# showlab/VideoSwap

Measured on NVIDIA H100. Metric: denoise-steps/sec, 16f 512^2 SD1.5 UNet3D (CFG UNet fwd + CFG combine + DDIM step), higher is better.
Workload: dtype f16

## Files before the change

videoswap_b200/csrc/common.cuh:

```cuda
#pragma once
#include <cuda.h>
#include <cuda_fp16.h>
#include <cuda_runtime.h>
#include <stdint.h>
#include <stdio.h>

namespace vs {

void set_error(const char* fmt, ...);
const char* last_error();

#define VS_CHECK_CUDA(expr)                                                                         \
  do {                                                                                              \
    cudaError_t _e = (expr);                                                                        \
    if (_e != cudaSuccess) {                                                                        \
      vs::set_error("%s:%d CUDA error %s: %s", __FILE__, __LINE__, #expr, cudaGetErrorString(_e)); \
      return 1;                                                                                     \
    }                                                                                               \
  } while (0)

#define VS_REQUIRE(cond, ...)                \
  do {                                       \
    if (!(cond)) {                           \
      vs::set_error(__VA_ARGS__);            \
// ... 41 lines not shown
  ProfScope(cudaStream_t st, int cat, double work, int nlaunch = 1, long long m = 0, int n = 0, int k = 0);
  ~ProfScope();
  cudaStream_t st_; int idx_;
};
void prof_enable(bool on);
void prof_reset();
int prof_collect(int cat, double* ms, double* work, long long* count);
int prof_dump(const char* path);
long long launch_count();
void count_launch(int n);

#ifdef __CUDACC__
__device__ __forceinline__ uint32_t smem_u32(const void* p) { return (uint32_t)__cvta_generic_to_shared(p); }

__device__ __forceinline__ void mbar_init(uint32_t bar, uint32_t count) {
  asm volatile("mbarrier.init.shared::cta.b64 [%0], %1;" ::"r"(bar), "r"(count) : "memory");
}
__device__ __forceinline__ void fence_barrier_init() {
  asm volatile("fence.mbarrier_init.release.cluster;" ::: "memory");
}
__device__ __forceinline__ void fence_proxy_async() { asm volatile("fence.proxy.async.shared::cta;" ::: "memory"); }
__device__ __forceinline__ void mbar_expect_tx(uint32_t bar, uint32_t bytes) {
  asm volatile("mbarrier.arrive.expect_tx.shared::cta.b64 _, [%0], %1;" ::"r"(bar), "r"(bytes) : "memory");
}
__device__ __forceinline__ void mbar_arrive(uint32_t bar) {
  asm volatile("mbarrier.arrive.shared::cta.b64 _, [%0];" ::"r"(bar) : "memory");
}
__device__ __forceinline__ bool mbar_try_wait(uint32_t bar, uint32_t parity) {
  uint32_t ok;
  asm volatile(
      "{\n\t.reg .pred p;\n\t"
      "mbarrier.try_wait.parity.shared::cta.b64 p, [%1], %2;\n\t"
      "selp.u32 %0, 1, 0, p;\n\t}"
      : "=r"(ok)
      : "r"(bar), "r"(parity)
      : "memory");
  return ok != 0;
}
__device__ __forceinline__ void mbar_wait(uint32_t bar, uint32_t parity) {
  if (mbar_try_wait(bar, parity)) return;
  uint32_t spins = 0;
  while (!mbar_try_wait(bar, parity)) {
    if (++spins > (1u << 25)) __trap();
  }
}

__device__ __forceinline__ void prefetch_tmap(const CUtensorMap* m) {
  asm volatile("prefetch.tensormap [%0];" ::"l"(reinterpret_cast<uint64_t>(m)) : "memory");
}
__device__ __forceinline__ void tma_load_2d(uint32_t dst, const CUtensorMap* m, uint32_t bar, int c0, int c1) {
  asm volatile(
      "cp.async.bulk.tensor.2d.shared::cluster.global.mbarrier::complete_tx::bytes [%0], [%1, {%3, %4}], [%2];"
      ::"r"(dst), "l"(reinterpret_cast<uint64_t>(m)), "r"(bar), "r"(c0), "r"(c1)
      : "memory");
}
__device__ __forceinline__ void tma_load_4d(uint32_t dst, const CUtensorMap* m, uint32_t bar, int c0, int c1, int c2,
                                            int c3) {
  asm volatile(
      "cp.async.bulk.tensor.4d.shared::cluster.global.mbarrier::complete_tx::bytes [%0], [%1, {%3, %4, %5, %6}], [%2];"
      ::"r"(dst), "l"(reinterpret_cast<uint64_t>(m)), "r"(bar), "r"(c0), "r"(c1), "r"(c2), "r"(c3)
      : "memory");
}

__device__ __forceinline__ bool elect_one() {
  uint32_t pred;
  asm volatile(
      "{\n\t.reg .pred P;\n\t"
      "elect.sync _|P, 0xffffffff;\n\t"
      "selp.u32 %0, 1, 0, P;\n\t}"
      : "=r"(pred));
  return pred != 0;
}

__device__ __forceinline__ uint32_t cluster_ctarank() {
  uint32_t r;
  asm volatile("mov.u32 %0, %%cluster_ctarank;" : "=r"(r));
  return r;
}
__device__ __forceinline__ void cluster_sync_all() {
  asm volatile("barrier.cluster.arrive.release.aligned;" ::: "memory");
  asm volatile("barrier.cluster.wait.acquire.aligned;" ::: "memory");
}
__device__ __forceinline__ uint32_t mapa_shared(uint32_t addr, uint32_t rank) {
  uint32_t r;
  asm volatile("mapa.shared::cluster.u32 %0, %1, %2;" : "=r"(r) : "r"(addr), "r"(rank));
  return r;
}
__device__ __forceinline__ void named_bar_sync(int id, int nthreads) {
  asm volatile("bar.sync %0, %1;" ::"r"(id), "r"(nthreads) : "memory");
}
__device__ __forceinline__ void named_bar_arrive(int id, int nthreads) {
  asm volatile("bar.arrive %0, %1;" ::"r"(id), "r"(nthreads) : "memory");
}

__device__ __forceinline__ void pdl_trigger() { asm volatile("griddepcontrol.launch_dependents;" ::: "memory"); }
__device__ __forceinline__ void pdl_wait() { asm volatile("griddepcontrol.wait;" ::: "memory"); }

template <int N>
__device__ __forceinline__ void setmaxnreg_dec() { asm volatile("setmaxnreg.dec.sync.aligned.u32 %0;" ::"n"(N)); }
template <int N>
__device__ __forceinline__ void setmaxnreg_inc() { asm volatile("setmaxnreg.inc.sync.aligned.u32 %0;" ::"n"(N)); }

__device__ __forceinline__ void wgmma_fence() { asm volatile("wgmma.fence.sync.aligned;" ::: "memory"); }
__device__ __forceinline__ void wgmma_commit() { asm volatile("wgmma.commit_group.sync.aligned;" ::: "memory"); }
template <int N>
__device__ __forceinline__ void wgmma_wait() { asm volatile("wgmma.wait_group.sync.aligned %0;" ::"n"(N) : "memory"); }
// ... 112 lines not shown
```

videoswap_b200/csrc/gemm.cu:

```cuda
#include <type_traits>

#include "common.cuh"
#include "kernels.h"

namespace vs {

namespace {

constexpr int BM = 128;
constexpr int WG_M = 64;
constexpr int BK = 64;
constexpr int A_STAGE_BYTES = BM * BK * 2;
constexpr uint64_t A_HALF_DESC = (WG_M * BK * 2) >> 4;
constexpr int GEMM_THREADS = 384;
constexpr int SMEM_LIMIT = 227 * 1024;
constexpr int EPI_COLS = 32;
constexpr int EPI_WARP_BYTES = 16 * 64;
constexpr int EPI_BYTES = 8 * EPI_WARP_BYTES;
constexpr int PRODUCER_REGS = 40, CONSUMER_REGS = 232;
enum { EPI_F_GEGLU = 1, EPI_F_RES = 2, EPI_F_RV = 4, EPI_F_LN = 8, EPI_F_LNOUT = 16, EPI_F_QGELU = 32 };

struct GemmParams {
  CUtensorMap tmA, tmA2, tmB;
  int M, N;
  int num_kb;
  int kb_per_tap;
  int kb_src1;
  int taps;
  int a_rank;
  int nimg, H, W, TH, TW, TN, tiles_x, tiles_y;
  int tap_x0, tap_y0, tap_w;
  int osy, osx, ooy, oox, OH, OW;
  int tw_log, thw_log;
  int m_tiles, n_tiles;
  const float* bias;
  const float* rowvec;
  int ldrv;
  int pix_per_batch;
  int rv_mod;
  const float2* ln_stats;
  const float* ln_u;
  const float2* ln_parts;
  int ln_nparts;
  float ln_inv_c;
  float2* ln_sums_out;
  const __half* residual;
  int ldr;
  __half* out;
  int ldc;
  int staged;
  int stages;
};

struct GemmParamsSub : GemmParams {
  CUtensorMap tmS[3];
  int sub_short;
};

struct GemmParamsS2 : GemmParams {
  CUtensorMap tmP[3];
};

template <int BN>
struct Cfg {
  static constexpr bool COOP = BN > 160;
  static constexpr int HALVES = COOP ? 1 : 2;
  static constexpr int B_STAGE_BYTES = BN * BK * 2;
  static constexpr int STAGE_BYTES = A_STAGE_BYTES + B_STAGE_BYTES;
  static constexpr int STAGES_RAW = (SMEM_LIMIT - 2048 - EPI_BYTES) / STAGE_BYTES;
  static constexpr int STAGES = STAGES_RAW > 12 ? 12 : STAGES_RAW;
  static constexpr int SMEM_BYTES = STAGES * STAGE_BYTES + EPI_BYTES + 1024  + 256 ;
  static_assert(B_STAGE_BYTES % 1024 == 0, "B stage must keep 1024-byte alignment for SWIZZLE_128B");
  static_assert(STAGES >= 3, "pipeline too shallow");
  static_assert(BN % 32 == 0 && BN <= 256, "wgmma N");
};

__device__ __forceinline__ uint32_t sw64_off(int row, int chunk) {
  return (uint32_t)(row * 64 + ((chunk ^ ((row >> 1) & 3)) << 4));
}

template <int BN, int EPI, typename Params>
__global__ void __launch_bounds__(GEMM_THREADS, 1) gemm_tc_kernel(const __grid_constant__ Params p) {
  using C = Cfg<BN>;
  constexpr bool SUB = std::is_same<Params, GemmParamsSub>::value;
  constexpr bool S2 = std::is_same<Params, GemmParamsS2>::value;
  constexpr bool GEGLU = (EPI & EPI_F_GEGLU) != 0, HAS_RES = (EPI & EPI_F_RES) != 0, HAS_RV = (EPI & EPI_F_RV) != 0;
  constexpr bool LN = (EPI & EPI_F_LN) != 0;
  constexpr bool LNOUT = (EPI & EPI_F_LNOUT) != 0;
  constexpr bool QGELU = (EPI & EPI_F_QGELU) != 0;
  extern __shared__ uint8_t smem_raw[];
  const uint32_t smem_base = (smem_u32(smem_raw) + 1023u) & ~1023u;
  const uint32_t epi_base = smem_base + C::STAGES * C::STAGE_BYTES;
  const uint32_t bar_base = epi_base + EPI_BYTES;
  auto full_bar = [&](int s) { return bar_base + 8u * s; };
  auto empty_bar = [&](int s) { return bar_base + 8u * (C::STAGES + s); };

  const int warp = threadIdx.x >> 5;
  const int lane = threadIdx.x & 31;
  const int wg = threadIdx.x >> 7;
  const int nst = (p.stages > 0 && p.stages < C::STAGES) ? p.stages : C::STAGES;
  const int total_tiles = p.m_tiles * p.n_tiles;

  if (threadIdx.x == 0) {
    prefetch_tmap(&p.tmA);
    prefetch_tmap(&p.tmB);
    if (p.kb_src1 < p.kb_per_tap) prefetch_tmap(&p.tmA2);
    if constexpr (SUB) {
      if (p.sub_short & 1) prefetch_tmap(&p.tmS[0]);
      if (p.sub_short & 2) prefetch_tmap(&p.tmS[1]);
      if (p.sub_short == 3) prefetch_tmap(&p.tmS[2]);
    }
    if constexpr (S2) {
      for (int k = 0; k < 3; ++k) prefetch_tmap(&p.tmP[k]);
    }
    for (int s = 0; s < C::STAGES; ++s) {
      mbar_init(full_bar(s), 1);
      mbar_init(empty_bar(s), C::COOP ? 8 : 4);
    }
    fence_barrier_init();
  }
  __syncthreads();
  pdl_trigger();
  pdl_wait();

  if (wg == 0) {
    setmaxnreg_dec<PRODUCER_REGS>();
    if (warp != 0) return;
    const int num_kb = p.num_kb, kb_per_tap = p.kb_per_tap, kb_src1 = p.kb_src1;
    const bool conv = p.a_rank == 4;
    const int tap_x0 = p.tap_x0, tap_x1 = p.tap_x0 + p.tap_w;
    bool short_y = false, short_x = false;
    if constexpr (SUB) { short_y = (p.sub_short & 1) != 0; short_x = (p.sub_short & 2) != 0; }
    uint32_t pr_s = 0, pr_ph = 0;
    for (int t = blockIdx.x; t < total_tiles; t += gridDim.x) {
      const int m_tile = t / p.n_tiles, n_tile = t % p.n_tiles;
      int x0 = 0, y0 = 0, i0 = 0;
      if (conv) {
        x0 = (m_tile % p.tiles_x) * p.TW;
        y0 = ((m_tile / p.tiles_x) % p.tiles_y) * p.TH;
        i0 = (m_tile / (p.tiles_x * p.tiles_y)) * p.TN;
      }
      const int n0 = n_tile * BN;
      const int m0 = m_tile * BM;
      int kcoord = 0;
      int dy = p.tap_y0, dx = tap_x0;
      int r = 0;
      for (int kb = 0; kb < num_kb; ++kb) {
        mbar_wait(empty_bar(pr_s), pr_ph ^ 1);
        if (elect_one()) {
          const uint32_t fb = full_bar(pr_s);
          const uint32_t a_dst = smem_base + pr_s * C::STAGE_BYTES;
          const bool first = r < kb_src1;
          const CUtensorMap* tm = first ? &p.tmA : &p.tmA2;
          if constexpr (SUB) {
            const bool sy = short_y && dy == p.tap_y0 + 2, sx = short_x && dx == tap_x0 + 2;
            if (sy || sx) tm = sy ? (sx ? &p.tmS[2] : &p.tmS[0]) : &p.tmS[1];
          }
          int ox = dx, oy = dy;
          if constexpr (S2) {
            const int par = ((dy & 1) << 1) | (dx & 1);
            if (par) tm = &p.tmP[par - 1];
            ox = dx >> 1; oy = dy >> 1;
          }
          const int c = (first ? r : r - kb_src1) * BK;
          mbar_expect_tx(fb, C::STAGE_BYTES);
          if (conv) tma_load_4d(a_dst, tm, fb, c, x0 + ox, y0 + oy, i0);
          else tma_load_2d(a_dst, tm, fb, c, m0);
          tma_load_2d(a_dst + A_STAGE_BYTES, &p.tmB, fb, kcoord, n0);
        }
        __syncwarp();
        kcoord += BK;
        if (++r == kb_per_tap) {
          r = 0;
          if (++dx == tap_x1) { dx = tap_x0; ++dy; }
        }
        if (++pr_s == (uint32_t)nst) { pr_s = 0; pr_ph ^= 1; }
      }
    }
    return;
  }

  setmaxnreg_inc<CONSUMER_REGS>();
  const int g = wg - 1;
  const int wq = warp & 3;
  const int q = lane & 3;
  const int rbase = 16 * wq + (lane >> 2);
  const uint32_t stage_buf = epi_base + (uint32_t)(warp - 4) * EPI_WARP_BYTES;
  const bool has_bias = p.bias != nullptr;
  const bool staged = p.staged != 0;
  const int num_kb = p.num_kb;
  auto tile_pixel = [&](int m_tile, int row) -> int {
    if (p.a_rank == 4) {
      const int x0 = (m_tile % p.tiles_x) * p.TW;
      const int y0 = ((m_tile / p.tiles_x) % p.tiles_y) * p.TH;
      const int i0 = (m_tile / (p.tiles_x * p.tiles_y)) * p.TN;
      const int ti = row >> p.thw_log, rem = row & ((1 << p.thw_log) - 1);
      const int y = y0 + (rem >> p.tw_log), x = x0 + (rem & (p.TW - 1)), img = i0 + ti;
      if constexpr (SUB) {
        const int oy = y * p.osy + p.ooy, ox = x * p.osx + p.oox;
        return ((img < p.nimg) && (y < p.H) && (x < p.W) && (oy < p.OH) && (ox < p.OW)) ? (img * p.OH + oy) * p.OW + ox : -1;
      }
      return ((img < p.nimg) && (y < p.H) && (x < p.W)) ? (img * p.OH + y * p.osy + p.ooy) * p.OW + x * p.osx + p.oox : -1;
    }
    const int px = m_tile * BM + row;
    return px < p.M ? px : -1;
  };

  const int bar_mine = 1 + g, bar_other = 2 - g;
  float acc[C::HALVES][BN / 2];
  uint32_t s = 0, ph = 0;
  for (int t = blockIdx.x, j = 0; t < total_tiles; t += gridDim.x, ++j) {
    const int m_tile = t / p.n_tiles, n_tile = t % p.n_tiles;
    if (!C::COOP && (j & 1) != g) {
      const uint32_t sn = s + (uint32_t)num_kb;
      ph ^= (sn / (uint32_t)nst) & 1u;
      s = sn % (uint32_t)nst;
      continue;
    }
    if (!C::COOP && j > 0) named_bar_sync(bar_mine, 256);
    uint32_t prev = 0;
    for (int kb = 0; kb < num_kb; ++kb) {
      mbar_wait(full_bar(s), ph);
      wgmma_fence();
      const uint32_t a_addr = smem_base + s * C::STAGE_BYTES;
      const uint64_t da = gmma_desc_sw128(a_addr) + (C::COOP ? (uint64_t)g * A_HALF_DESC : 0);
      const uint64_t db = gmma_desc_sw128(a_addr + A_STAGE_BYTES);
#pragma unroll
      for (int k = 0; k < BK / 16; ++k) {
#pragma unroll
        for (int hh = 0; hh < C::HALVES; ++hh)
          wgmma_ss<BN>(acc[hh], da + hh * A_HALF_DESC + 2 * k, db + 2 * k, (kb | k) != 0 ? 1u : 0u);
      }
      wgmma_commit();
      if (kb > 0) {
        wgmma_wait<1>();
        if (lane == 0) mbar_arrive(empty_bar(prev));
      }
      prev = s;
      if (++s == (uint32_t)nst) { s = 0; ph ^= 1; }
    }
    if (!C::COOP && t + (int)gridDim.x < total_tiles) named_bar_arrive(bar_other, 256);
    wgmma_wait<0>();
    if (lane == 0) mbar_arrive(empty_bar(prev));

    const int n0 = n_tile * BN;
#pragma unroll
    for (int hh = 0; hh < C::HALVES; ++hh) {
      const int r0 = WG_M * (C::COOP ? g : hh) + rbase;
      int pix[2];
      pix[0] = tile_pixel(m_tile, r0);
      pix[1] = tile_pixel(m_tile, r0 + 8);
      const float* rv[2] = {nullptr, nullptr};
      if (HAS_RV || !staged) {
#pragma unroll
        for (int h = 0; h < 2; ++h) {
          if (p.rowvec != nullptr && pix[h] >= 0) {
            int ri = pix[h] / p.pix_per_batch;
            if (p.rv_mod > 0) ri %= p.rv_mod;
            rv[h] = p.rowvec + (long long)ri * p.ldrv + n0;
          }
        }
      }
      if (staged) {
        constexpr int OC = GEGLU ? BN / 2 : BN;
        const int oc0 = n_tile * OC;
        const int nsub = (p.N - n0 < BN ? (GEGLU ? (p.N - n0) / 2 : p.N - n0) : OC) / EPI_COLS;
        float la[2] = {1.f, 1.f}, lb[2] = {0.f, 0.f};
        if (LN) {
#pragma unroll
          for (int h = 0; h < 2; ++h) {
            if (pix[h] < 0) continue;
            if (p.ln_nparts > 0) {
              float S = 0.f, Q = 0.f;
              for (int k = 0; k < p.ln_nparts; ++k) {
                const float2 v = __ldg(p.ln_parts + (long long)k * p.M + pix[h]);
                S += v.x; Q += v.y;
              }
              const float mean = S * p.ln_inv_c;
              la[h] = rsqrtf(fmaxf(fmaf(-mean, mean, Q * p.ln_inv_c), 0.f) + 1e-5f);
              lb[h] = -mean * la[h];
            } else {
              const float2 st2 = __ldg(p.ln_stats + pix[h]);
              la[h] = st2.x; lb[h] = st2.y;
            }
          }
        }
        float rs[2] = {0.f, 0.f}, rq[2] = {0.f, 0.f};
        __half* orow[2];
        const __half* rrow[2];
#pragma unroll
        for (int h = 0; h < 2; ++h) {
          const long long px = pix[h] >= 0 ? pix[h] : 0;
          orow[h] = p.out + px * p.ldc + oc0 + q * 8;
          rrow[h] = HAS_RES ? p.residual + px * p.ldr + oc0 + q * 8 : nullptr;
        }
#pragma unroll
        for (int sb = 0; sb < OC / EPI_COLS; ++sb) {
          if (sb >= nsub) break;
          uint4 rr[2];
          if (HAS_RES) {
#pragma unroll
            for (int h = 0; h < 2; ++h) rr[h] = __ldg(reinterpret_cast<const uint4*>(rrow[h] + sb * EPI_COLS));
          }
#pragma unroll
          for (int jj = 0; jj < 4; ++jj) {
            const int j = 4 * sb + jj;
            const int c = 8 * j + 2 * q;
            float2 b = has_bias ? __ldg(reinterpret_cast<const float2*>(p.bias + n0 + c)) : make_float2(0.f, 0.f);
            float2 u = LN ? __ldg(reinterpret_cast<const float2*>(p.ln_u + n0 + c)) : make_float2(0.f, 0.f);
            float2 bg = make_float2(0.f, 0.f), ug = make_float2(0.f, 0.f);
            if (GEGLU) {
              bg = __ldg(reinterpret_cast<const float2*>(p.bias + n0 + BN / 2 + c));
              if (LN) ug = __ldg(reinterpret_cast<const float2*>(p.ln_u + n0 + BN / 2 + c));
            }
#pragma unroll
            for (int h = 0; h < 2; ++h) {
              float f0 = acc[hh][4 * j + 2 * h], f1 = acc[hh][4 * j + 2 * h + 1];
              if (GEGLU) {
                float g0 = acc[hh][4 * (j + BN / 16) + 2 * h], g1 = acc[hh][4 * (j + BN / 16) + 2 * h + 1];
                float bv0 = b.x, bv1 = b.y, bg0 = bg.x, bg1 = bg.y;
                if (LN) {
                  bv0 = fmaf(lb[h], u.x, bv0); bv1 = fmaf(lb[h], u.y, bv1);
                  bg0 = fmaf(lb[h], ug.x, bg0); bg1 = fmaf(lb[h], ug.y, bg1);
                  f0 *= la[h]; f1 *= la[h]; g0 *= la[h]; g1 *= la[h];
                }
                f0 = (f0 + bv0) * gelu_sig(g0 + bg0);
                f1 = (f1 + bv1) * gelu_sig(g1 + bg1);
              } else {
                if (LN) {
                  f0 = fmaf(la[h], f0, fmaf(lb[h], u.x, b.x));
                  f1 = fmaf(la[h], f1, fmaf(lb[h], u.y, b.y));
                } else if (has_bias) {
                  f0 += b.x; f1 += b.y;
                }
                if (HAS_RV && rv[h] != nullptr) {
                  const float2 r2 = __ldg(reinterpret_cast<const float2*>(rv[h] + c));
                  f0 += r2.x; f1 += r2.y;
                }
                if constexpr (QGELU) {
                  f0 = quick_gelu_f(f0); f1 = quick_gelu_f(f1);
                }
              }
              const __half2 hv = __floats2half2_rn(f0, f1);
              asm volatile("st.shared.b32 [%0], %1;" ::"r"(stage_buf + sw64_off((lane >> 2) + 8 * h, jj) + 4 * q),
                           "r"(*reinterpret_cast<const uint32_t*>(&hv)) : "memory");
            }
          }
          __syncwarp();
#pragma unroll
          for (int h = 0; h < 2; ++h) {
            uint4 o;
            asm volatile("ld.shared.v4.b32 {%0,%1,%2,%3}, [%4];" : "=r"(o.x), "=r"(o.y), "=r"(o.z), "=r"(o.w)
                         : "r"(stage_buf + sw64_off((lane >> 2) + 8 * h, q)));
            if (HAS_RES) {
              __half2* oh = reinterpret_cast<__half2*>(&o);
              const __half2* rh = reinterpret_cast<const __half2*>(&rr[h]);
#pragma unroll
              for (int t = 0; t < 4; ++t) oh[t] = __hadd2(oh[t], rh[t]);
            }
            if (pix[h] >= 0) *reinterpret_cast<uint4*>(orow[h] + sb * EPI_COLS) = o;
            if (LNOUT) {
              const __half2* oh = reinterpret_cast<const __half2*>(&o);
              const float2 a = __half22float2(oh[0]), b2 = __half22float2(oh[1]), c2 = __half22float2(oh[2]), d2 = __half22float2(oh[3]);
              rs[h] += ((a.x + a.y) + (b2.x + b2.y)) + ((c2.x + c2.y) + (d2.x + d2.y));
              float q0 = fmaf(a.x, a.x, a.y * a.y), q1 = fmaf(b2.x, b2.x, b2.y * b2.y);
              float q2 = fmaf(c2.x, c2.x, c2.y * c2.y), q3 = fmaf(d2.x, d2.x, d2.y * d2.y);
              rq[h] += (q0 + q1) + (q2 + q3);
            }
          }
          __syncwarp();
        }
        if (LNOUT) {
#pragma unroll
          for (int h = 0; h < 2; ++h) {
            rs[h] += __shfl_xor_sync(0xffffffffu, rs[h], 1); rq[h] += __shfl_xor_sync(0xffffffffu, rq[h], 1);
            rs[h] += __shfl_xor_sync(0xffffffffu, rs[h], 2); rq[h] += __shfl_xor_sync(0xffffffffu, rq[h], 2);
            if (q == 0 && pix[h] >= 0) p.ln_sums_out[(long long)n_tile * p.M + pix[h]] = make_float2(rs[h], rq[h]);
          }
        }
      } else {
#pragma unroll
        for (int j = 0; j < BN / 8; ++j) {
#pragma unroll
          for (int e = 0; e < 4; ++e) {
            const int h = e >> 1, c = 8 * j + 2 * q + (e & 1), n = n0 + c;
            if (n < p.N && pix[h] >= 0) {
              float f = acc[hh][4 * j + e];
              if (has_bias) f += p.bias[n];
              if (rv[h]) f += rv[h][c];
              __half y = __float2half_rn(f);
              if (p.residual) y = __hadd(y, p.residual[(long long)pix[h] * p.ldr + n]);
              p.out[(long long)pix[h] * p.ldc + n] = y;
            }
          }
        }
      }
    }
  }
}

struct ConvTile { int tw, th, tn; };

ConvTile pick_conv_tile(int nimg, int H, int W) {
  ConvTile best{1, 1, BM};
  long long best_cost = -1;
  for (int tw = 1; tw <= BM; tw *= 2) {
    for (int th = 1; tw * th <= BM; th *= 2) {
      const int tn = BM / (tw * th);
      if (tw > 256 || th > 256 || tn > 256) continue;
      const long long cost = (long long)((W + tw - 1) / tw) * tw * ((H + th - 1) / th) * th * ((nimg + tn - 1) / tn) * tn;
      if (best_cost < 0 || cost < best_cost || (cost == best_cost && tw > best.tw)) {
        best_cost = cost;
        best = ConvTile{tw, th, tn};
      }
    }
  }
  return best;
}

template <int BN, int EPI, typename Params = GemmParams>
int launch(cudaStream_t st, const Params& p) {
  using C = Cfg<BN>;
  static bool configured = false;
  if (!configured) {
    VS_CHECK_CUDA(cudaFuncSetAttribute(gemm_tc_kernel<BN, EPI, Params>, cudaFuncAttributeMaxDynamicSharedMemorySize, C::SMEM_BYTES));
    configured = true;
  }
  const int total = p.m_tiles * p.n_tiles;
  int ctas = num_sms();
  const int cap = get_option("gemm_ctas");
  if (cap > 0 && cap < ctas) ctas = cap;
  return launch_pdl(gemm_tc_kernel<BN, EPI, Params>, dim3(total < ctas ? total : ctas), dim3(GEMM_THREADS), C::SMEM_BYTES, st, 1, p);
}

template <int BN>
int launch_linear(cudaStream_t st, const GemmParams& p) {
  const int epi = (p.residual ? EPI_F_RES : 0) | (p.rowvec ? EPI_F_RV : 0) | ((p.ln_stats || p.ln_parts) ? EPI_F_LN : 0) |
                  (p.ln_sums_out ? EPI_F_LNOUT : 0);
  switch (epi) {
    case EPI_F_LNOUT: return launch<BN, EPI_F_LNOUT>(st, p);
    case EPI_F_LNOUT | EPI_F_RES: return launch<BN, EPI_F_LNOUT | EPI_F_RES>(st, p);
    case EPI_F_LN: return launch<BN, EPI_F_LN>(st, p);
    case EPI_F_LN | EPI_F_RV: return launch<BN, EPI_F_LN | EPI_F_RV>(st, p);
    case 0: return launch<BN, 0>(st, p);
    case EPI_F_RES: return launch<BN, EPI_F_RES>(st, p);
    case EPI_F_RV: return launch<BN, EPI_F_RV>(st, p);
    case EPI_F_RES | EPI_F_RV: return launch<BN, EPI_F_RES | EPI_F_RV>(st, p);
    default: set_error("gemm_tc: unsupported epilogue combination 0x%x", epi); return 2;
  }
}

int pick_bn(int m_tiles, int N, int num_kb) {
  if (N <= 64) return 64;
  int best = 128;
  long long best_cost = -1;
  const int cand[3] = {128, 160, 256};
  for (int i = 0; i < 3; ++i) {
    const int bn = cand[i];
    if (bn != 128 && N % bn != 0) continue;
    const long long tiles = (long long)m_tiles * ((N + bn - 1) / bn);
    const long long waves = (tiles + num_sms() - 1) / num_sms();
    const long long cost = waves * (16 + bn / 8);
    if (best_cost < 0 || cost < best_cost || (cost == best_cost && num_kb >= 40)) {
      best_cost = cost;
      best = bn;
    }
  }
  return best;
}

int ilog2(int v) { int l = 0; while ((1 << l) < v) ++l; return l; }

}

int gemm_n_tiles(const GemmArgs& a) {
  if (a.taps != 1) return 0;
  int bn = a.force_bn;
  if (a.mode == EPI_GEGLU) bn = 2 * kGegluGranule;
  else if (bn == 0) bn = pick_bn((a.M + BM - 1) / BM, a.N, (a.K1 + BK - 1) / BK + a.K2 / BK);
  return (a.N + bn - 1) / bn;
}

int gemm_tc(cudaStream_t st, const GemmArgs& a) {
  VS_REQUIRE(a.A && a.Bw && a.out, "gemm_tc: null pointer");
  VS_REQUIRE(a.taps == 1 || a.taps == 9 || a.taps == 4, "gemm_tc: taps must be 1, 9 (3x3) or 4 (sub-pixel)");
  VS_REQUIRE(a.K1 % 8 == 0 && a.K2 % 8 == 0, "gemm_tc: K must be a multiple of 8 (TMA 16-byte strides)");
  VS_REQUIRE((long long)a.M * (a.ldc > a.ldr ? a.ldc : a.ldr) < (1LL << 40) && a.M < (1 << 30), "gemm_tc: M too large");
  const bool two = a.A2 != nullptr && a.K2 > 0;
  if (two || a.taps != 1) VS_REQUIRE(a.K1 % BK == 0 && a.K2 % BK == 0, "gemm_tc: concat/conv sources need C %% 64 == 0 (got %d,%d)", a.K1, a.K2);
  GemmParamsSub ps;
  memset(&ps, 0, sizeof(ps));
  GemmParams& p = ps;
  GemmParamsS2 p2;
  memset(&p2, 0, sizeof(p2));
  const bool sub = a.taps == 4;
  const int OH = sub && a.OH > 0 ? a.OH : 2 * a.H, OW = sub && a.OW > 0 ? a.OW : 2 * a.W;
  const int sub_ty = sub && a.sub_py == 0 && (OH & 1) ? 3 : 2, sub_tx = sub && a.sub_px == 0 && (OW & 1) ? 3 : 2;
  if (sub) VS_REQUIRE((OH == 2 * a.H || OH == 2 * a.H - 1) && (OW == 2 * a.W || OW == 2 * a.W - 1),
                      "gemm_tc: sub-pixel output %dx%d is not 2x (or 2x - 1) of the %dx%d input", OH, OW, a.H, a.W);
  const int ntaps = sub ? sub_ty * sub_tx : a.taps;
  const int Ktap = a.K1 + (two ? a.K2 : 0);
// ... 66 lines not shown
      }
    }
    if (two) {
      const uint64_t dims[4] = {(uint64_t)a.K2, (uint64_t)a.W, (uint64_t)a.H, (uint64_t)a.nimg};
      const uint64_t str[3] = {(uint64_t)a.lda2 * 2, (uint64_t)a.lda2 * 2 * a.W, (uint64_t)a.lda2 * 2 * a.W * a.H};
      if (make_tmap_f16(&p.tmA2, a.A2, 4, dims, str, box, 1)) return 3;
    }
  } else {
    p.a_rank = 2;
    p.m_tiles = (a.M + BM - 1) / BM;
    const uint32_t box[2] = {BK, BM};
    {
      const uint64_t dims[2] = {(uint64_t)a.K1, (uint64_t)a.M};
      const uint64_t str[1] = {(uint64_t)a.lda1 * 2};
      if (make_tmap_f16(&p.tmA, a.A, 2, dims, str, box, 1)) return 3;
    }
    if (two) {
      const uint64_t dims[2] = {(uint64_t)a.K2, (uint64_t)a.M};
      const uint64_t str[1] = {(uint64_t)a.lda2 * 2};
      if (make_tmap_f16(&p.tmA2, a.A2, 2, dims, str, box, 1)) return 3;
    }
  }

  int bn = a.force_bn;
  if (a.mode == EPI_GEGLU) {
    bn = 2 * kGegluGranule;
    VS_REQUIRE(a.N % bn == 0, "gemm_tc: GEGLU needs N %% %d == 0 (N=%d)", bn, a.N);
    VS_REQUIRE(a.bias != nullptr && a.residual == nullptr && a.rowvec == nullptr, "gemm_tc: GEGLU takes a bias only");
  } else if (bn == 0) {
    bn = pick_bn(p.m_tiles, a.N, p.num_kb);
  }
  VS_REQUIRE(bn == 64 || bn == 128 || bn == 160 || bn == 256, "gemm_tc: unsupported BLOCK_N %d", bn);
  p.n_tiles = (a.N + bn - 1) / bn;
  {
    const uint64_t dims[2] = {(uint64_t)Ktot, (uint64_t)a.N};
    const uint64_t str[1] = {(uint64_t)Ktot * 2};
    const uint32_t box[2] = {BK, (uint32_t)bn};
    if (make_tmap_f16(&p.tmB, a.Bw, 2, dims, str, box, 1)) return 3;
  }
  const int out_cols = (a.mode == EPI_GEGLU) ? a.N / 2 : a.N;
  p.staged = (out_cols % EPI_COLS == 0) && (a.ldc % 8 == 0) && ((reinterpret_cast<uintptr_t>(a.out) & 15) == 0) &&
             (!a.residual || ((a.ldr % 8 == 0) && ((reinterpret_cast<uintptr_t>(a.residual) & 15) == 0))) &&
             (!a.bias || (reinterpret_cast<uintptr_t>(a.bias) & 15) == 0) &&
             (!a.rowvec || ((reinterpret_cast<uintptr_t>(a.rowvec) & 15) == 0 && p.ldrv % 4 == 0));
  if (a.mode == EPI_QUICK_GELU)
    VS_REQUIRE(a.taps == 1 && p.staged && a.residual == nullptr && a.rowvec == nullptr && !a.ln_stats && !a.ln_parts &&
               a.ln_sums_out == nullptr && (bn == 128 || bn == 256),
               "gemm_tc: the quick-GELU epilogue takes a plain GEMM with a bias only, N %% 32 == 0 and BLOCK_N 128 / 256 (got %d)", bn);
  if (!p.staged) VS_REQUIRE(a.mode == EPI_LINEAR, "gemm_tc: GEGLU output needs 32-column aligned, 16-byte strided rows");
  if (a.ln_stats || a.ln_parts) VS_REQUIRE(p.staged && (reinterpret_cast<uintptr_t>(a.ln_u) & 15) == 0, "gemm_tc: folded LayerNorm needs the staged epilogue");
  if (a.ln_sums_out) VS_REQUIRE(p.staged, "gemm_tc: row statistics output needs the staged epilogue (N %% 32 == 0, aligned rows)");
  ProfScope prof(st, a.taps != 1 ? PC_CONV : PC_GEMM, 2.0 * a.M * (double)a.N * Ktot, 1, a.M, a.N, Ktot);
  if (a.mode == EPI_GEGLU) {
    if (p.ln_stats || p.ln_parts) return launch<256, EPI_F_GEGLU | EPI_F_LN>(st, p);
    return launch<256, EPI_F_GEGLU>(st, p);
  }
  if (a.mode == EPI_QUICK_GELU) return bn == 256 ? launch<256, EPI_F_QGELU>(st, p) : launch<128, EPI_F_QGELU>(st, p);
  if (s2) {
    VS_REQUIRE(a.residual == nullptr && a.rowvec == nullptr && a.ln_sums_out == nullptr && p.staged,
               "gemm_tc: the stride-2 conv takes a bias only and needs N %% 32 == 0");
    static_cast<GemmParams&>(p2) = p;
    switch (bn) {
      case 64: return launch<64, 0, GemmParamsS2>(st, p2);
      case 128: return launch<128, 0, GemmParamsS2>(st, p2);
      case 256: return launch<256, 0, GemmParamsS2>(st, p2);
      default: return launch<160, 0, GemmParamsS2>(st, p2);
    }
  }
  if (sub && ((OH | OW) & 1)) {
    VS_REQUIRE(a.residual == nullptr && a.rowvec == nullptr && p.staged, "gemm_tc: an odd-sized sub-pixel conv takes a bias only");
    switch (bn) {
      case 64: return launch<64, 0, GemmParamsSub>(st, ps);
      case 128: return launch<128, 0, GemmParamsSub>(st, ps);
      case 256: return launch<256, 0, GemmParamsSub>(st, ps);
      default: return launch<160, 0, GemmParamsSub>(st, ps);
    }
  }
  switch (bn) {
    case 64: return launch_linear<64>(st, p);
    case 128: return launch_linear<128>(st, p);
    case 256: return launch_linear<256>(st, p);
    default: return launch_linear<160>(st, p);
  }
}

static const __half* subpixel_panel(const __half* w3x3, const __half* wsub, int cout, int cin, int py, int px, bool odd_y,
                                    bool odd_x) {
  const bool ty3 = py == 0 && odd_y, tx3 = px == 0 && odd_x;
  const size_t tap = (size_t)cout * cin;
  if (ty3 && tx3) return w3x3;
  if (ty3) return wsub + (16 + 6 * px) * tap;
  if (tx3) return wsub + (28 + 6 * py) * tap;
  return wsub + (size_t)(2 * py + px) * 4 * tap;
}

int upsample_conv3x3(cudaStream_t st, const __half* x, int nimg, int H, int W, int C, const __half* w3x3, const __half* wsub,
                     const float* bias, int cout, int OH, int OW, __half* out) {
  VS_REQUIRE((OH == 2 * H || OH == 2 * H - 1) && (OW == 2 * W || OW == 2 * W - 1),
             "upsample_conv3x3: output %dx%d is not 2x (or 2x - 1) of the %dx%d input", OH, OW, H, W);
  VS_REQUIRE(w3x3 != nullptr || ((OH & 1) == 0 && (OW & 1) == 0), "upsample_conv3x3: odd output sizes need the 3x3 panel");
  for (int par = 0; par < 4; ++par) {
    GemmArgs g;
    g.A = x; g.K1 = C; g.lda1 = C; g.Bw = subpixel_panel(w3x3, wsub, cout, C, par >> 1, par & 1, OH & 1, OW & 1); g.taps = 4;
    g.sub_py = par >> 1; g.sub_px = par & 1; g.OH = OH; g.OW = OW; g.nimg = nimg; g.H = H; g.W = W; g.M = nimg * H * W;
    g.N = cout; g.bias = bias; g.out = out; g.ldc = cout;
    if (int e = gemm_tc(st, g)) return e;
  }
  return 0;
}

}
```

videoswap_b200/csrc/runtime.cu:

```cuda
#include <stdarg.h>
#include <string.h>

#include <mutex>

#include "common.cuh"
#include "kernels.h"

namespace vs {

static thread_local char g_err[1024] = "";

void set_error(const char* fmt, ...) {
  va_list ap;
  va_start(ap, fmt);
  vsnprintf(g_err, sizeof(g_err), fmt, ap);
  va_end(ap);
}
const char* last_error() { return g_err; }

typedef CUresult (*EncodeTiledFn)(CUtensorMap*, CUtensorMapDataType, cuuint32_t, void*, const cuuint64_t*,
                                  const cuuint64_t*, const cuuint32_t*, const cuuint32_t*, CUtensorMapInterleave,
                                  CUtensorMapSwizzle, CUtensorMapL2promotion, CUtensorMapFloatOOBfill);

static EncodeTiledFn get_encode() {
// ... 36 lines not shown
                   CU_TENSOR_MAP_L2_PROMOTION_L2_256B, CU_TENSOR_MAP_FLOAT_OOB_FILL_NONE);
  VS_REQUIRE(r == CUDA_SUCCESS, "cuTensorMapEncodeTiled failed with CUresult %d (rank %d dims %llu,%llu box %u,%u)",
             (int)r, rank, (unsigned long long)dims[0], (unsigned long long)dims[1], box[0], box[1]);
  return 0;
}

int num_sms() {
  static int n = 0;
  if (n == 0) {
    int dev = 0;
    cudaGetDevice(&dev);
    cudaDeviceGetAttribute(&n, cudaDevAttrMultiProcessorCount, dev);
    if (n <= 0) n = 132;
  }
  return n;
}

}

#include <atomic>
#include <vector>

namespace vs {

static std::atomic<long long> g_launches{0};
static bool g_prof_on = false;
struct ProfEntry { cudaEvent_t a, b; int cat; double work; long long m; int n, k; };
static std::vector<ProfEntry> g_prof;
static std::vector<std::pair<cudaEvent_t, cudaEvent_t>> g_pool;

void count_launch(int n) { g_launches.fetch_add(n, std::memory_order_relaxed); }
long long launch_count() { return g_launches.load(); }

ProfScope::ProfScope(cudaStream_t st, int cat, double work, int nlaunch, long long m, int n, int k) : st_(st), idx_(-1) {
  count_launch(nlaunch);
  if (!g_prof_on) return;
  ProfEntry e;
  if (!g_pool.empty()) { e.a = g_pool.back().first; e.b = g_pool.back().second; g_pool.pop_back(); }
  else { cudaEventCreate(&e.a); cudaEventCreate(&e.b); }
  e.cat = cat; e.work = work; e.m = m; e.n = n; e.k = k;
  cudaEventRecord(e.a, st);
  idx_ = (int)g_prof.size();
  g_prof.push_back(e);
}
ProfScope::~ProfScope() {
  if (idx_ >= 0) cudaEventRecord(g_prof[idx_].b, st_);
}

struct Option { const char* name; int value; };
static Option g_options[] = {
    {"attn_tc", 1},
    {"gemm_stages", 0},
    {"gemm_ctas", 0},
    {"ln_fold", 1},
    {"ln_fuse", 1},
    {"tattn_vst", 1},
    {"gn_fused", 1},
    {"gn_stats_v2", 0},
    {"subpixel", 1},
    {"pdl", 1},
};
int set_option(const char* name, int value) {
  for (Option& o : g_options)
    if (strcmp(name, o.name) == 0) { o.value = value; return 0; }
  set_error("unknown option '%s'", name);
  return 2;
}
int get_option(const char* name) {
  for (const Option& o : g_options)
    if (strcmp(name, o.name) == 0) return o.value;
  return 0;
}

int prof_dump(const char* path) {
  struct Agg { int cat; long long m; int n, k; double work, ms; long long count; };
  std::vector<Agg> aggs;
  for (auto& e : g_prof) {
    if (cudaEventSynchronize(e.b) != cudaSuccess) { set_error("profile: event sync failed"); return 1; }
    float ms = 0.f;
    cudaEventElapsedTime(&ms, e.a, e.b);
    Agg* hit = nullptr;
    for (auto& a : aggs)
      if (a.cat == e.cat && a.m == e.m && a.n == e.n && a.k == e.k && a.work == e.work) { hit = &a; break; }
    if (!hit) { aggs.push_back(Agg{e.cat, e.m, e.n, e.k, e.work, 0.0, 0}); hit = &aggs.back(); }
    hit->ms += ms;
    hit->count += 1;
  }
  FILE* f = fopen(path, "w");
  if (!f) { set_error("cannot open %s", path); return 2; }
  fprintf(f, "category,m,n,k,work_per_launch,launches,total_ms\n");
  for (auto& a : aggs) fprintf(f, "%d,%lld,%d,%d,%.6g,%lld,%.4f\n", a.cat, a.m, a.n, a.k, a.work, a.count, a.ms);
  fclose(f);
  return 0;
}

void prof_enable(bool on) { g_prof_on = on; }
void prof_reset() {
  for (auto& e : g_prof) g_pool.push_back({e.a, e.b});
  g_prof.clear();
}
int prof_collect(int cat, double* ms, double* work, long long* count) {
  double t = 0, w = 0; long long n = 0;
  for (auto& e : g_prof) {
    if (e.cat != cat) continue;
    if (cudaEventSynchronize(e.b) != cudaSuccess) { set_error("profile: event sync failed"); return 1; }
    float m = 0.f;
// ... 9 lines not shown
```

Before: 10.94.

## Prefetch GEMM epilogue operands into double-buffered shared slots via bulk copies

Adds a dedicated producer warp that uses TMA and bulk async copies to load each tile's epilogue operands (bias, residual tile, LayerNorm vectors and row statistics, row vectors) into double-buffered shared-memory slots, guarded by mbarriers. Consumer warpgroups then read these from shared memory instead of issuing scattered global loads during the epilogue, so those loads overlap with the mainloop of the current tile. In exchange the slots take shared memory, which can lower the pipeline stage count, and add barrier waits. The path is gated by a new option that defaults on and covers only certain linear and GEGLU epilogue combinations.

After: 11.39, median of 6. 4.1% higher.

```diff
diff --git a/videoswap_b200/csrc/common.cuh b/videoswap_b200/csrc/common.cuh
--- a/videoswap_b200/csrc/common.cuh
+++ b/videoswap_b200/csrc/common.cuh
@@ -117,6 +117,12 @@
   asm volatile(
       "cp.async.bulk.tensor.2d.shared::cluster.global.mbarrier::complete_tx::bytes [%0], [%1, {%3, %4}], [%2];"
       ::"r"(dst), "l"(reinterpret_cast<uint64_t>(m)), "r"(bar), "r"(c0), "r"(c1)
+      : "memory");
+}
+__device__ __forceinline__ void bulk_load(uint32_t dst, const void* src, uint32_t bytes, uint32_t bar) {
+  asm volatile(
+      "cp.async.bulk.shared::cluster.global.mbarrier::complete_tx::bytes [%0], [%1], %2, [%3];"
+      ::"r"(dst), "l"(reinterpret_cast<uint64_t>(src)), "r"(bytes), "r"(bar)
       : "memory");
 }
 __device__ __forceinline__ void tma_load_4d(uint32_t dst, const CUtensorMap* m, uint32_t bar, int c0, int c1, int c2,
diff --git a/videoswap_b200/csrc/gemm.cu b/videoswap_b200/csrc/gemm.cu
--- a/videoswap_b200/csrc/gemm.cu
+++ b/videoswap_b200/csrc/gemm.cu
@@ -61,17 +61,37 @@
   CUtensorMap tmP[3];
 };
 
-template <int BN>
+constexpr int LN_MAX_PARTS = 8;
+struct GemmParamsEpi : GemmParams {
+  CUtensorMap tmR;
+};
+
+template <int BN, int EPI>
+struct EpiSlot {
+  static constexpr bool RES = (EPI & EPI_F_RES) != 0, LN = (EPI & EPI_F_LN) != 0, RV = (EPI & EPI_F_RV) != 0;
+  static constexpr int RES_BYTES = RES ? BM * BN * 2 : 0;
+  static constexpr int BIAS_OFF = RES_BYTES;
+  static constexpr int U_OFF = BIAS_OFF + BN * 4;
+  static constexpr int RV_OFF = U_OFF + (LN ? BN * 4 : 0);
+  static constexpr int LNR_OFF = RV_OFF + (RV ? 2 * BN * 4 : 0);
+  static constexpr int END = LNR_OFF + (LN ? LN_MAX_PARTS * BM * 8 : 0);
+  static constexpr int BYTES = RES ? (END + 1023) / 1024 * 1024 : (END + 127) / 128 * 128;
+};
+
+template <int BN, int SLOT_BYTES = 0>
 struct Cfg {
   static constexpr bool COOP = BN > 160;
   static constexpr int HALVES = COOP ? 1 : 2;
   static constexpr int B_STAGE_BYTES = BN * BK * 2;
   static constexpr int STAGE_BYTES = A_STAGE_BYTES + B_STAGE_BYTES;
-  static constexpr int STAGES_RAW = (SMEM_LIMIT - 2048 - EPI_BYTES) / STAGE_BYTES;
+  static constexpr int STAGES_RAW = SLOT_BYTES ? (SMEM_LIMIT - 1024 - 256 - EPI_BYTES - 2 * SLOT_BYTES) / STAGE_BYTES
+                                               : (SMEM_LIMIT - 2048 - EPI_BYTES) / STAGE_BYTES;
   static constexpr int STAGES = STAGES_RAW > 12 ? 12 : STAGES_RAW;
-  static constexpr int SMEM_BYTES = STAGES * STAGE_BYTES + EPI_BYTES + 1024  + 256 ;
+  static constexpr int SMEM_BYTES =
+      STAGES * STAGE_BYTES + EPI_BYTES + 2 * SLOT_BYTES + 1024  + 256 ;
   static_assert(B_STAGE_BYTES % 1024 == 0, "B stage must keep 1024-byte alignment for SWIZZLE_128B");
   static_assert(STAGES >= 3, "pipeline too shallow");
+  static_assert(SMEM_BYTES <= SMEM_LIMIT, "shared memory");
   static_assert(BN % 32 == 0 && BN <= 256, "wgmma N");
 };
 
@@ -81,9 +101,12 @@
 
 template <int BN, int EPI, typename Params>
 __global__ void __launch_bounds__(GEMM_THREADS, 1) gemm_tc_kernel(const __grid_constant__ Params p) {
-  using C = Cfg<BN>;
   constexpr bool SUB = std::is_same<Params, GemmParamsSub>::value;
   constexpr bool S2 = std::is_same<Params, GemmParamsS2>::value;
+  constexpr bool SLOT = std::is_same<Params, GemmParamsEpi>::value;
+  using ES = EpiSlot<BN, EPI>;
+  using C = Cfg<BN, SLOT ? ES::BYTES : 0>;
+  static_assert(!SLOT || ((C::COOP == ((EPI & EPI_F_GEGLU) != 0)) && (EPI & EPI_F_QGELU) == 0), "epilogue slots: ping-pong linears and cooperative GEGLUs");
   constexpr bool GEGLU = (EPI & EPI_F_GEGLU) != 0, HAS_RES = (EPI & EPI_F_RES) != 0, HAS_RV = (EPI & EPI_F_RV) != 0;
   constexpr bool LN = (EPI & EPI_F_LN) != 0;
   constexpr bool LNOUT = (EPI & EPI_F_LNOUT) != 0;
@@ -91,9 +114,12 @@
   extern __shared__ uint8_t smem_raw[];
   const uint32_t smem_base = (smem_u32(smem_raw) + 1023u) & ~1023u;
   const uint32_t epi_base = smem_base + C::STAGES * C::STAGE_BYTES;
-  const uint32_t bar_base = epi_base + EPI_BYTES;
+  const uint32_t slot_base = epi_base + EPI_BYTES;
+  const uint32_t bar_base = slot_base + (SLOT ? 2 * ES::BYTES : 0);
   auto full_bar = [&](int s) { return bar_base + 8u * s; };
   auto empty_bar = [&](int s) { return bar_base + 8u * (C::STAGES + s); };
+  auto slot_full = [&](int g) { return bar_base + 8u * (2 * C::STAGES + g); };
+  auto slot_empty = [&](int g) { return bar_base + 8u * (2 * C::STAGES + 2 + g); };
 
   const int warp = threadIdx.x >> 5;
   const int lane = threadIdx.x & 31;
@@ -113,6 +139,13 @@
     if constexpr (S2) {
       for (int k = 0; k < 3; ++k) prefetch_tmap(&p.tmP[k]);
     }
+    if constexpr (SLOT) {
+      if (ES::RES) prefetch_tmap(&p.tmR);
+      for (int g = 0; g < 2; ++g) {
+        mbar_init(slot_full(g), 1);
+        mbar_init(slot_empty(g), C::COOP ? 8 : 4);
+      }
+    }
     for (int s = 0; s < C::STAGES; ++s) {
       mbar_init(full_bar(s), 1);
       mbar_init(empty_bar(s), C::COOP ? 8 : 4);
@@ -125,6 +158,47 @@
 
   if (wg == 0) {
     setmaxnreg_dec<PRODUCER_REGS>();
+    if constexpr (SLOT) {
+      if (warp == 1) {
+        for (int t = blockIdx.x, j = 0; t < total_tiles; t += gridDim.x, ++j) {
+          const int g = j & 1;
+          mbar_wait(slot_empty(g), ((j >> 1) & 1) ^ 1);
+          if (elect_one()) {
+            const int m_tile = t / p.n_tiles, n_tile = t % p.n_tiles;
+            const int n0 = n_tile * BN, m0 = m_tile * BM;
+            const int ncols = p.N - n0 < BN ? p.N - n0 : BN;
+            const int parts = p.ln_nparts > 0 ? p.ln_nparts : 1;
+            const int rows = p.M - m0 < BM ? p.M - m0 : BM;
+            const int last = m0 + rows - 1;
+            int rv0 = m0 / p.pix_per_batch, rv1 = last / p.pix_per_batch;
+            const int nrv = rv1 != rv0 ? 2 : 1;
+            if (p.rv_mod > 0) { rv0 %= p.rv_mod; rv1 %= p.rv_mod; }
+            const uint32_t sb = slot_base + (uint32_t)g * ES::BYTES, fb = slot_full(g);
+            uint32_t bytes = p.bias != nullptr ? ncols * 4u : 0u;
+            if (ES::RES) bytes += (uint32_t)(ncols / EPI_COLS) * (BM * 64);
+            if (ES::LN) bytes += ncols * 4u + (uint32_t)(parts * rows) * 8u;
+            if (ES::RV) bytes += (uint32_t)nrv * ncols * 4u;
+            mbar_expect_tx(fb, bytes);
+            if (p.bias != nullptr) bulk_load(sb + ES::BIAS_OFF, p.bias + n0, ncols * 4u, fb);
+            if constexpr (ES::RES) {
+              for (int c = 0; c < ncols / EPI_COLS; ++c) tma_load_2d(sb + c * (BM * 64), &p.tmR, fb, n0 + c * EPI_COLS, m0);
+            }
+            if constexpr (ES::LN) {
+              bulk_load(sb + ES::U_OFF, p.ln_u + n0, ncols * 4u, fb);
+              const float2* src = p.ln_nparts > 0 ? p.ln_parts : p.ln_stats;
+              for (int k = 0; k < parts; ++k)
+                bulk_load(sb + ES::LNR_OFF + k * (BM * 8), src + (long long)k * p.M + m0, rows * 8u, fb);
+            }
+            if constexpr (ES::RV) {
+              bulk_load(sb + ES::RV_OFF, p.rowvec + (long long)rv0 * p.ldrv + n0, ncols * 4u, fb);
+              if (nrv == 2) bulk_load(sb + ES::RV_OFF + BN * 4, p.rowvec + (long long)rv1 * p.ldrv + n0, ncols * 4u, fb);
+            }
+          }
+          __syncwarp();
+        }
+        return;
+      }
+    }
     if (warp != 0) return;
     const int num_kb = p.num_kb, kb_per_tap = p.kb_per_tap, kb_src1 = p.kb_src1;
     const bool conv = p.a_rank == 4;
@@ -187,7 +261,7 @@
   const int rbase = 16 * wq + (lane >> 2);
   const uint32_t stage_buf = epi_base + (uint32_t)(warp - 4) * EPI_WARP_BYTES;
   const bool has_bias = p.bias != nullptr;
-  const bool staged = p.staged != 0;
+  const bool staged = SLOT || p.staged != 0;
   const int num_kb = p.num_kb;
   auto tile_pixel = [&](int m_tile, int row) -> int {
     if (p.a_rank == 4) {
@@ -242,6 +316,9 @@
     if (!C::COOP && t + (int)gridDim.x < total_tiles) named_bar_arrive(bar_other, 256);
     wgmma_wait<0>();
     if (lane == 0) mbar_arrive(empty_bar(prev));
+    const int js = j & 1;
+    const uint8_t* slot = smem_raw + (slot_base + (uint32_t)js * ES::BYTES - smem_u32(smem_raw));
+    if constexpr (SLOT) mbar_wait(slot_full(js), (uint32_t)(j >> 1) & 1u);
 
     const int n0 = n_tile * BN;
 #pragma unroll
@@ -251,7 +328,13 @@
       pix[0] = tile_pixel(m_tile, r0);
       pix[1] = tile_pixel(m_tile, r0 + 8);
       const float* rv[2] = {nullptr, nullptr};
-      if (HAS_RV || !staged) {
+      if (SLOT && HAS_RV) {
+#pragma unroll
+        for (int h = 0; h < 2; ++h) {
+          const int d = pix[h] >= 0 ? pix[h] / p.pix_per_batch - (m_tile * BM) / p.pix_per_batch : 0;
+          rv[h] = reinterpret_cast<const float*>(slot + ES::RV_OFF) + d * BN;
+        }
+      } else if (HAS_RV || !staged) {
 #pragma unroll
         for (int h = 0; h < 2; ++h) {
           if (p.rowvec != nullptr && pix[h] >= 0) {
@@ -270,17 +353,18 @@
 #pragma unroll
           for (int h = 0; h < 2; ++h) {
             if (pix[h] < 0) continue;
+            const float2* lnr = reinterpret_cast<const float2*>(slot + ES::LNR_OFF) + r0 + 8 * h;
             if (p.ln_nparts > 0) {
               float S = 0.f, Q = 0.f;
               for (int k = 0; k < p.ln_nparts; ++k) {
-                const float2 v = __ldg(p.ln_parts + (long long)k * p.M + pix[h]);
+                const float2 v = SLOT ? lnr[k * BM] : __ldg(p.ln_parts + (long long)k * p.M + pix[h]);
                 S += v.x; Q += v.y;
               }
               const float mean = S * p.ln_inv_c;
               la[h] = rsqrtf(fmaxf(fmaf(-mean, mean, Q * p.ln_inv_c), 0.f) + 1e-5f);
               lb[h] = -mean * la[h];
             } else {
-              const float2 st2 = __ldg(p.ln_stats + pix[h]);
+              const float2 st2 = SLOT ? lnr[0] : __ldg(p.ln_stats + pix[h]);
               la[h] = st2.x; lb[h] = st2.y;
             }
           }
@@ -298,7 +382,11 @@
         for (int sb = 0; sb < OC / EPI_COLS; ++sb) {
           if (sb >= nsub) break;
           uint4 rr[2];
-          if (HAS_RES) {
+          if (SLOT && HAS_RES) {
+#pragma unroll
+            for (int h = 0; h < 2; ++h)
+              rr[h] = *reinterpret_cast<const uint4*>(slot + sb * (BM * 64) + sw64_off(r0 + 8 * h, q));
+          } else if (HAS_RES) {
 #pragma unroll
             for (int h = 0; h < 2; ++h) rr[h] = __ldg(reinterpret_cast<const uint4*>(rrow[h] + sb * EPI_COLS));
           }
@@ -306,12 +394,23 @@
           for (int jj = 0; jj < 4; ++jj) {
             const int j = 4 * sb + jj;
             const int c = 8 * j + 2 * q;
-            float2 b = has_bias ? __ldg(reinterpret_cast<const float2*>(p.bias + n0 + c)) : make_float2(0.f, 0.f);
-            float2 u = LN ? __ldg(reinterpret_cast<const float2*>(p.ln_u + n0 + c)) : make_float2(0.f, 0.f);
+            float2 b = make_float2(0.f, 0.f), u = make_float2(0.f, 0.f);
+            if constexpr (SLOT) {
+              if (has_bias) b = *reinterpret_cast<const float2*>(slot + ES::BIAS_OFF + 4 * c);
+              if (LN) u = *reinterpret_cast<const float2*>(slot + ES::U_OFF + 4 * c);
+            } else {
+              if (has_bias) b = __ldg(reinterpret_cast<const float2*>(p.bias + n0 + c));
+              if (LN) u = __ldg(reinterpret_cast<const float2*>(p.ln_u + n0 + c));
+            }
             float2 bg = make_float2(0.f, 0.f), ug = make_float2(0.f, 0.f);
             if (GEGLU) {
-              bg = __ldg(reinterpret_cast<const float2*>(p.bias + n0 + BN / 2 + c));
-              if (LN) ug = __ldg(reinterpret_cast<const float2*>(p.ln_u + n0 + BN / 2 + c));
+              if constexpr (SLOT) {
+                bg = *reinterpret_cast<const float2*>(slot + ES::BIAS_OFF + 4 * (BN / 2 + c));
+                if (LN) ug = *reinterpret_cast<const float2*>(slot + ES::U_OFF + 4 * (BN / 2 + c));
+              } else {
+                bg = __ldg(reinterpret_cast<const float2*>(p.bias + n0 + BN / 2 + c));
+                if (LN) ug = __ldg(reinterpret_cast<const float2*>(p.ln_u + n0 + BN / 2 + c));
+              }
             }
 #pragma unroll
             for (int h = 0; h < 2; ++h) {
@@ -334,7 +433,8 @@
                   f0 += b.x; f1 += b.y;
                 }
                 if (HAS_RV && rv[h] != nullptr) {
-                  const float2 r2 = __ldg(reinterpret_cast<const float2*>(rv[h] + c));
+                  const float2 r2 = SLOT ? *reinterpret_cast<const float2*>(rv[h] + c)
+                                         : __ldg(reinterpret_cast<const float2*>(rv[h] + c));
                   f0 += r2.x; f1 += r2.y;
                 }
                 if constexpr (QGELU) {
@@ -342,8 +442,11 @@
                 }
               }
               const __half2 hv = __floats2half2_rn(f0, f1);
-              asm volatile("st.shared.b32 [%0], %1;" ::"r"(stage_buf + sw64_off((lane >> 2) + 8 * h, jj) + 4 * q),
-                           "r"(*reinterpret_cast<const uint32_t*>(&hv)) : "memory");
+              const uint32_t sa = stage_buf + sw64_off((lane >> 2) + 8 * h, jj) + 4 * q;
+              if constexpr (SLOT)
+                asm volatile("st.shared.b32 [%0], %1;" ::"r"(sa), "r"(*reinterpret_cast<const uint32_t*>(&hv)));
+              else
+                asm volatile("st.shared.b32 [%0], %1;" ::"r"(sa), "r"(*reinterpret_cast<const uint32_t*>(&hv)) : "memory");
             }
           }
           __syncwarp();
@@ -395,6 +498,10 @@
           }
         }
       }
+    }
+    if constexpr (SLOT) {
+      __syncwarp();
+      if (lane == 0) mbar_arrive(slot_empty(js));
     }
   }
 }
@@ -420,7 +527,7 @@
 
 template <int BN, int EPI, typename Params = GemmParams>
 int launch(cudaStream_t st, const Params& p) {
-  using C = Cfg<BN>;
+  using C = Cfg<BN, std::is_same<Params, GemmParamsEpi>::value ? EpiSlot<BN, EPI>::BYTES : 0>;
   static bool configured = false;
   if (!configured) {
     VS_CHECK_CUDA(cudaFuncSetAttribute(gemm_tc_kernel<BN, EPI, Params>, cudaFuncAttributeMaxDynamicSharedMemorySize, C::SMEM_BYTES));
@@ -447,6 +554,45 @@
     case EPI_F_RV: return launch<BN, EPI_F_RV>(st, p);
     case EPI_F_RES | EPI_F_RV: return launch<BN, EPI_F_RES | EPI_F_RV>(st, p);
     default: set_error("gemm_tc: unsupported epilogue combination 0x%x", epi); return 2;
+  }
+}
+
+template <int BN>
+int launch_linear_slot(cudaStream_t st, const GemmParams& p, const GemmArgs& a) {
+  const bool geglu = a.mode == EPI_GEGLU;
+  if (get_option("gemm_epi_slot") == 0 || a.taps != 1 || (a.mode != EPI_LINEAR && !geglu) || !p.staged || p.num_kb > 10)
+    return -1;
+  const int epi = (p.residual ? EPI_F_RES : 0) | (p.rowvec ? EPI_F_RV : 0) | ((p.ln_stats || p.ln_parts) ? EPI_F_LN : 0) |
+                  (p.ln_sums_out ? EPI_F_LNOUT : 0) | (geglu ? EPI_F_GEGLU : 0);
+  if (geglu ? (BN != 256 || (epi & ~EPI_F_LN) != EPI_F_GEGLU)
+            : (BN == 256 || (epi != EPI_F_RES && epi != EPI_F_LNOUT && epi != (EPI_F_LNOUT | EPI_F_RES) &&
+                             epi != EPI_F_LN && epi != (EPI_F_LN | EPI_F_RV))))
+    return -1;
+  GemmParamsEpi pe;
+  memset(&pe, 0, sizeof(pe));
+  static_cast<GemmParams&>(pe) = p;
+  if (p.rowvec && !(p.pix_per_batch >= BM || p.pix_per_batch == BM / 2)) return -1;
+  if (epi & EPI_F_LN) {
+    const void* rows = p.ln_parts ? static_cast<const void*>(p.ln_parts) : static_cast<const void*>(p.ln_stats);
+    const int parts = p.ln_parts ? p.ln_nparts : 1;
+    if (parts > LN_MAX_PARTS || (reinterpret_cast<uintptr_t>(rows) & 15) != 0 || (p.M & 1) != 0) return -1;
+  }
+  if (epi & EPI_F_RES) {
+    const uint64_t dims[2] = {(uint64_t)p.N, (uint64_t)p.M};
+    const uint64_t str[1] = {(uint64_t)p.ldr * 2};
+    const uint32_t box[2] = {EPI_COLS, BM};
+    if (make_tmap_f16(&pe.tmR, p.residual, 2, dims, str, box, 2)) return 3;
+  }
+  if constexpr (BN == 256) {
+    return epi == EPI_F_GEGLU ? launch<BN, EPI_F_GEGLU>(st, pe) : launch<BN, EPI_F_GEGLU | EPI_F_LN>(st, pe);
+  } else {
+    switch (epi) {
+      case EPI_F_RES: return launch<BN, EPI_F_RES>(st, pe);
+      case EPI_F_LNOUT: return launch<BN, EPI_F_LNOUT>(st, pe);
+      case EPI_F_LNOUT | EPI_F_RES: return launch<BN, EPI_F_LNOUT | EPI_F_RES>(st, pe);
+      case EPI_F_LN: return launch<BN, EPI_F_LN>(st, pe);
+      default: return launch<BN, EPI_F_LN | EPI_F_RV>(st, pe);
+    }
   }
 }
 
@@ -619,6 +765,7 @@
   if (a.ln_sums_out) VS_REQUIRE(p.staged, "gemm_tc: row statistics output needs the staged epilogue (N %% 32 == 0, aligned rows)");
   ProfScope prof(st, a.taps != 1 ? PC_CONV : PC_GEMM, 2.0 * a.M * (double)a.N * Ktot, 1, a.M, a.N, Ktot);
   if (a.mode == EPI_GEGLU) {
+    if (const int e = launch_linear_slot<256>(st, p, a); e >= 0) return e;
     if (p.ln_stats || p.ln_parts) return launch<256, EPI_F_GEGLU | EPI_F_LN>(st, p);
     return launch<256, EPI_F_GEGLU>(st, p);
   }
@@ -642,6 +789,10 @@
       case 256: return launch<256, 0, GemmParamsSub>(st, ps);
       default: return launch<160, 0, GemmParamsSub>(st, ps);
     }
+  }
+  if (bn == 128 || bn == 160) {
+    const int e = bn == 128 ? launch_linear_slot<128>(st, p, a) : launch_linear_slot<160>(st, p, a);
+    if (e >= 0) return e;
   }
   switch (bn) {
     case 64: return launch_linear<64>(st, p);
diff --git a/videoswap_b200/csrc/runtime.cu b/videoswap_b200/csrc/runtime.cu
--- a/videoswap_b200/csrc/runtime.cu
+++ b/videoswap_b200/csrc/runtime.cu
@@ -112,6 +112,7 @@
     {"attn_tc", 1},
     {"gemm_stages", 0},
     {"gemm_ctas", 0},
+    {"gemm_epi_slot", 1},
     {"ln_fold", 1},
     {"ln_fuse", 1},
     {"tattn_vst", 1},
```
